# penn-pal-lab/robot_aware_control

Hardware: AMD Instinct MI355X
Metric: SVG train frames/sec + CEM candidate-rollouts/sec, 64x64 (higher is better)
Workload: dtype fp32 (conv operands as two fp16 parts = 22 significant bits, fp32 accumulate; see fp32_exact)

## Files before the change

### include/rac_hip.h

```cpp
#ifndef RAC_HIP_H
#define RAC_HIP_H

#include <stddef.h>
#include <stdint.h>

#ifdef __cplusplus
extern "C" {
#endif

#define RAC_OK 0
#define RAC_EINVAL (-1)
#define RAC_ELAUNCH (-2)

#define RAC_ABI_VERSION 12

int rac_version(void);
const char* rac_device_arch(void);
const char* rac_last_error(void);

enum {
  RAC_CONV_FWD = 0,
  RAC_CONV_DGRAD = 1,
  RAC_CONV_WGRAD = 2
};
// ... 41 lines not shown
typedef struct rac_frag_job {
  const float* w;
  const uint32_t* w_amax;
  uint16_t* parts;
  int64_t part_stride;
  int32_t Cout, Cin, ksize, transposed;
  int64_t block_begin;
} rac_frag_job;
int64_t rac_absmax_blocks(int64_t n);
int64_t rac_weight_frag_blocks(int32_t Cout, int32_t Cin, int32_t ksize);
int rac_absmax_multi(const rac_absmax_job* jobs, int32_t n_jobs, int64_t total_blocks, void* stream);
int rac_weight_frag_split_multi(const rac_frag_job* jobs, int32_t n_jobs, int64_t total_blocks, void* stream);
int rac_conv2d_split_supported(int32_t H, int32_t W, int32_t ksize, int32_t Cin, int32_t Cout, int32_t a_split);
int rac_conv2d_fwd_split(const rac_conv_args* a, const uint32_t* a_amax0, const uint32_t* a_amax1,
                         int64_t w_part_stride, int32_t w_cin, const uint32_t* w_amax, uint32_t* out_amax, void* stream);
int rac_conv2d_fwd_split_pool_ok(const rac_conv_args* a, int32_t w_cin);
int rac_convlstm_cell_fwd_split(const rac_conv_args* a, const uint32_t* a_amax0, const uint32_t* a_amax1,
                                int64_t w_part_stride, int32_t w_cin, const uint32_t* w_amax, const float* c_prev,
                                float* h_out, float* c_out, void* stream);

#define RAC_WGRAD_MAX_STEPS 16
typedef struct rac_wgrad_args {
  int32_t B, H, W;
  int32_t ksize, Cin, Cout, a_split;
  int32_t T;
  int32_t nsplit;
  int32_t accumulate;
  const float* dy[RAC_WGRAD_MAX_STEPS];
  const float* x0[RAC_WGRAD_MAX_STEPS];
  const float* x1[RAC_WGRAD_MAX_STEPS];
// ... 287 lines not shown
```

### robot_aware_control_amd/_lib.py

```python
from __future__ import annotations

import ctypes as C
import os

import torch

_HERE = os.path.dirname(os.path.abspath(__file__))
LIB_PATH = os.environ.get("RAC_HIP_LIB") or os.path.join(_HERE, "librac_hip.so")

i32, i64, f32, vp = C.c_int32, C.c_int64, C.c_float, C.c_void_p


class ConvArgs(C.Structure):
    _fields_ = [
        ("mode", i32), ("B", i32), ("H", i32), ("W", i32), ("ksize", i32), ("Cin", i32), ("Cout", i32),
        ("act", i32), ("split_k", i32), ("accumulate", i32), ("a_split", i32), ("o_split", i32),
        ("slab_stride", i64),
        ("a0", vp), ("a1", vp), ("w", vp), ("out0", vp), ("out1", vp),
        ("bias", vp), ("scale", vp), ("shift", vp), ("stats", vp),
        ("stats_rows", i64), ("a0_up", i32), ("amax_per_image", i32),
    ]


WGRAD_MAX_STEPS = 16
# ... 66 lines not shown
        ("all_ky", i32), ("col_segments", i32),
    ]


_SIGS = {
    "rac_conv2d": [C.POINTER(ConvArgs), vp],
    "rac_absmax": [vp, i64, vp, i64, vp, vp],
    "rac_absmax_rows": [vp, i64, i64, vp, vp],
    "rac_weight_frag_split": [vp, vp, vp, i32, i32, i32, i32, i64, vp],
    "rac_absmax_blocks": [i64],
    "rac_weight_frag_blocks": [i32, i32, i32],
    "rac_absmax_multi": [vp, i32, i64, vp],
    "rac_weight_frag_split_multi": [vp, i32, i64, vp],
    "rac_conv2d_split_supported": [i32, i32, i32, i32, i32, i32],
    "rac_conv2d_fwd_split": [C.POINTER(ConvArgs), vp, vp, i64, i32, vp, vp, vp],
    "rac_conv2d_fwd_split_pool_ok": [C.POINTER(ConvArgs), i32],
    "rac_convlstm_cell_fwd_split": [C.POINTER(ConvArgs), vp, vp, i64, i32, vp, vp, vp, vp, vp],
    "rac_conv2d_wgrad_split": [C.POINTER(WgradArgs), vp],
    "rac_split_steps": [C.POINTER(vp), C.POINTER(vp), i32, i64, C.POINTER(vp), i32, vp],
    "rac_slab_accumulate": [vp, i32, i64, vp, i64, vp],
    "rac_bn_finalize": [vp, i64, vp, vp, vp, vp, f32, f32, i32, vp, vp, vp, vp, i32, i32, vp],
    "rac_affine_act": [vp, vp, vp, i32, vp, i64, i32, i32, vp, vp],
    "rac_bn_apply_act": [vp, i64, vp, vp, vp, vp, f32, f32, i32, vp, i32, vp, vp, vp, vp, vp, i64, i32, i32, vp, vp],
    "rac_bn_bwd_reduce": [vp, vp, vp, vp, vp, vp, vp, i64, i32, i32, vp],
    "rac_bn_bwd_apply": [vp, vp, vp, vp, vp, vp, vp, vp, vp, vp, i64, i32, i32, vp, vp],
    "rac_maxpool2_fwd": [vp, vp, i32, i32, i32, i32, vp],
    "rac_maxpool2_bwd": [vp, vp, vp, i32, i32, i32, i32, vp],
    "rac_upsample2_fwd": [vp, vp, i32, i32, i32, i32, vp],
    "rac_upsample2_bwd": [vp, vp, i32, i32, i32, i32, vp],
    "rac_tilecat_fwd": [vp, i32, vp, i32, vp, i32, vp, i32, vp, i32, i32, vp, i32, i32, vp, i32, vp],
# ... 134 lines not shown
```

### robot_aware_control_amd/csrc/rac_split16.hip

```cpp
#include <math.h>
#include <stdlib.h>

#include <type_traits>

#include "rac_common.h"

namespace rac {

typedef _Float16 f16x8 __attribute__((ext_vector_type(8)));
typedef _Float16 f16x4 __attribute__((ext_vector_type(4)));
typedef unsigned int u32x4 __attribute__((ext_vector_type(4)));
typedef unsigned int u32x2 __attribute__((ext_vector_type(2)));
typedef __amdgpu_buffer_rsrc_t rsrc_t;

constexpr unsigned OOB = 0xFFFFFFF0u;
constexpr int SBN = 128, SBK = 32;

__device__ __forceinline__ const void* uniform_ptr(const void* p) {
  unsigned long long v = reinterpret_cast<unsigned long long>(p);
  unsigned lo = __builtin_amdgcn_readfirstlane((unsigned)v);
  unsigned hi = __builtin_amdgcn_readfirstlane((unsigned)(v >> 32));
  return reinterpret_cast<const void*>(((unsigned long long)hi << 32) | lo);
}
__device__ __forceinline__ rsrc_t make_rsrc(const void* p, unsigned bytes) {
// ... 45 lines not shown
  double* stats;
  long stats_rows;
  int M, N, HW, P, taps, cchunks, nchunks, cps;
  int w_nchunks;
  int xcd_group;
  int tile_m;
  int n_store;
  int a0_up;
  const float* lstm_c_prev;
  float *lstm_h, *lstm_c;
  int lstm_g;
  int per_image;
  int seg_w, seg_h, seg_tx, seg_tpi;
  float* pool_out;
  int pool_bpr;
};

struct SegOrigin {
  int img, y0, x0, m0;
};
__device__ __forceinline__ SegOrigin seg_origin(const Conv16P& p, int bx) {
  SegOrigin o;
  o.img = bx / p.seg_tpi;
  const int r = bx - o.img * p.seg_tpi;
  const int ty = r / p.seg_tx;
  o.y0 = ty * p.seg_h;
  o.x0 = (r - ty * p.seg_tx) * p.seg_w;
  o.m0 = (o.img * p.H + o.y0) * p.W + o.x0;
  return o;
}
// ... 86 lines not shown
        const float sc = pre ? pre[nb][1] : (p.scale ? p.scale[ncol0 + nb * 16 + lr] : 1.f);
        const float sh = pre ? pre[nb][2] : (p.scale ? p.shift[ncol0 + nb * 16 + lr] : 0.f);
#pragma unroll
        for (int r = 0; r < 4; ++r) {
          float v = acc[mb][nb][r] * iav[mb][r] * iw + bias;
          v = v * sc + sh;
          v = v > 0.f ? v : slope * v;
          if (SIG) v = sigmoid_acc(v);
          __builtin_amdgcn_raw_buffer_store_b32(__builtin_bit_cast(unsigned, v), dst, (int)voff[r] + nb * 64, 0, 0);
          mxb[mb] = max(mxb[mb], absbits(v));
        }
      }
    }
    return;
  }
#pragma unroll
  for (int nb = 0; nb < NBLK; ++nb) {
    const int n = ncol0 + nb * 16 + lr;
    const bool nok = n < NS;
    const int nc = nok ? n : 0;
    const float bias = pre ? pre[nb][0] : (p.bias ? p.bias[nc] : 0.f);
    const float sc = pre ? pre[nb][1] : (p.scale ? p.scale[nc] : 1.f);
    const float sh = pre ? pre[nb][2] : (p.scale ? p.shift[nc] : 0.f);
    float s1 = 0.f, s2 = 0.f;
#pragma unroll
    for (int mb = 0; mb < MBLK; ++mb) {
      if (mb0 + mb >= nmb) continue;
#pragma unroll
      for (int r = 0; r < 4; ++r) {
        const int rl = 4 * lq + r;
        const int m = ym_hw ? m0 + (rl >> 3) * ym_hw + (mb0 + mb) * 8 + (rl & 7) : seg_row_pixel(p, m0, (mb0 + mb) * 16) + rl;
        const bool ok = nok & (m < p.M);
        float v = acc[mb][nb][r] * iav[mb][r] * iw + bias;
        const float vs = ok ? v : 0.f;
        s1 += vs;
        s2 += vs * vs;
        v = v * sc + sh;
        v = v > 0.f ? v : slope * v;
        if (SIG) v = sigmoid_acc(v);
        if (ok) {
          p.out0[(long)m * NS + n] = v;
          mxb[mb] = max(mxb[mb], absbits(v));
        }
      }
    }
    if (p.stats) {
      s1 += __shfl_xor(s1, 16);
      s2 += __shfl_xor(s2, 16);
      s1 += __shfl_xor(s1, 32);
      s2 += __shfl_xor(s2, 32);
      if (lq == 0 && nok) {
        double* sg = p.stats + (p.stats_rows ? (long)(m0 / p.stats_rows) * 2 * NS : 0L);
        atomicAdd(sg + n, (double)s1);
        atomicAdd(sg + NS + n, (double)s2);
      }
    }
  }
}

template <int MBLK, int NBLK>
__device__ __forceinline__ void conv16_epilogue(const Conv16P& p, const f32x4 (&acc)[MBLK][NBLK], int m0, int mb0, int nmb,
                                                int ncol0, int bz, float ia, float iw, const float (*pre)[3] = nullptr,
                                                const float* ia_rows = nullptr, unsigned* out_amax = nullptr,
                                                int ym_hw = 0) {
  const int lane = threadIdx.x & 63, lr = lane & 15, lq = lane >> 4;
  const int NS = p.n_store;
  if (p.split_k > 1) {
    float* dst = p.out0 + (long)bz * p.slab_stride;
#pragma unroll
    for (int nb = 0; nb < NBLK; ++nb) {
      const int n = ncol0 + nb * 16 + lr;
#pragma unroll
      for (int mb = 0; mb < MBLK; ++mb) {
        if (mb0 + mb >= nmb) continue;
#pragma unroll
        for (int r = 0; r < 4; ++r) {
          const int rl = 4 * lq + r;
          const int m = ym_hw ? m0 + (rl >> 3) * ym_hw + (mb0 + mb) * 8 + (rl & 7) : seg_row_pixel(p, m0, (mb0 + mb) * 16) + rl;
          if ((n < NS) & (m < p.M)) dst[(long)m * NS + n] = acc[mb][nb][r] * ia * iw;
        }
      }
    }
    return;
  }
  unsigned mxb[MBLK];
  if (p.act == RAC_ACT_SIGMOID)
    conv16_epilogue_body<1>(p, acc, m0, mb0, nmb, ncol0, ia, iw, pre, ia_rows, mxb, ym_hw);
  else
    conv16_epilogue_body<0>(p, acc, m0, mb0, nmb, ncol0, ia, iw, pre, ia_rows, mxb, ym_hw);
  if (!out_amax) return;
  if (ia_rows && ym_hw) {
    unsigned mx = 0;
#pragma unroll
    for (int mb = 0; mb < MBLK; ++mb) mx = max(mx, mxb[mb]);
    const int img0 = m0 / ym_hw;
    amax_commit(lq < 2 ? mx : 0u, out_amax + img0);
    if (m0 + ym_hw < p.M) amax_commit(lq >= 2 ? mx : 0u, out_amax + img0 + 1);
    return;
  }
// ... 1201 lines not shown
          __syncthreads();
          cur ^= 1;
        }
        if (tap < 8 || more) {
#pragma unroll
          for (int t = 0; t < HB; ++t) read_frag(t, (tap + 1) % 9, cur * abuf);
        }
        __builtin_amdgcn_sched_barrier(0);
#pragma unroll
        for (int t = HB; t < MB; ++t)
#pragma unroll
          for (int nb = 0; nb < NB; ++nb) acc[t][nb] = mma3(fa[t], fb[nb], acc[t][nb]);
      }
    }
    const int img = p.per_image ? cur_t.m0 / p.HW : 0;
    conv16_epilogue(p, acc, cur_t.m0, wm * MB, nmb, n0 + wn * NT * 32, 0, pow2f(-cur_t.ka), pow2f(-kw), pre, nullptr,
                    p.out_amax ? p.out_amax + img : nullptr);
    if (!has_next) break;
    cur ^= 1;
    cur_t = nxt_t;
    bx = next_bx;
  }
}

__global__ __launch_bounds__(256) void absmax_kernel(const float4* x0, long n0v, const float4* x1, long n1v,
                                                     unsigned* amax) {
  __shared__ unsigned sh[4];
  unsigned m = 0;
  const long stride = (long)gridDim.x * blockDim.x;
  for (long i = (long)blockIdx.x * blockDim.x + threadIdx.x; i < n0v + n1v; i += stride) {
    const float4 v = i < n0v ? x0[i] : x1[i - n0v];
// ... 882 lines not shown

static int env_int(const char* name, int dflt) {
  const char* e = getenv(name);
  return e ? atoi(e) : dflt;
}

extern "C" int rac_conv2d_split_supported(int32_t H, int32_t W, int32_t ksize, int32_t Cin, int32_t Cout, int32_t a_split) {
  if (H <= 0 || W <= 0 || ksize < 3 || ksize > 5 || !(ksize & 1) || Cin % 32 || Cout % 32) return 0;
  if (a_split > 0 && a_split < Cin && a_split % 32) return 0;
  const int HW = H * W;
  if (HW <= 128) return ((128 / HW) * HW) % 16 == 0;
  if (rows_fit(H, W, ksize)) return 1;
  return ksize == 3 && W >= 64 && W % 16 == 0 && H % 8 == 0;
}

static int conv16_launch(const rac_conv_args* a, const uint32_t* a_amax0, const uint32_t* a_amax1, int64_t w_part_stride,
                         int32_t w_cin, const uint32_t* w_amax, uint32_t* out_amax, const float* lstm_c_prev, float* lstm_h,
                         float* lstm_c, void* stream, bool pool_query = false) {
  RAC_REQUIRE(a && a->mode == RAC_CONV_FWD, "rac_conv2d_fwd_split: forward mode only");
  RAC_REQUIRE(a->B > 0 && a->H > 0 && a->W > 0 && a->Cin > 0 && a->Cout > 0 && a->a0 && a->w && (a->out0 || lstm_h) && a_amax0 &&
                  w_amax,
              "rac_conv2d_fwd_split: bad args");
  const int a_split = (a->a1 && a->a_split > 0 && a->a_split < a->Cin) ? a->a_split : a->Cin;
  const int n_rows = (a->Cout + 31) / 32 * 32;
  RAC_REQUIRE(rac_conv2d_split_supported(a->H, a->W, a->ksize, a->Cin, n_rows, a_split),
              "rac_conv2d_fwd_split: shape not supported (k 3 or 5, channel counts %% 32 == 0, whole images or whole "
              "image rows per 128-pixel tile): use rac_conv2d");
  Conv16P p{};
  p.B = a->B, p.H = a->H, p.W = a->W, p.ks = a->ksize, p.pad = a->ksize / 2;
  p.Cin = a->Cin, p.Cout = a->Cout, p.act = a->act;
  p.split_k = a->split_k > 1 ? a->split_k : 1;
  p.slab_stride = a->slab_stride;
  p.a0 = a->a0, p.a1 = a->a1;
// ... 12 lines not shown
  p.per_image = a->amax_per_image ? 1 : 0;
  RAC_REQUIRE(!p.per_image || (p.split_k == 1 && (p.HW > 128 || p.HW % 16 == 0)),
              "rac_conv2d_fwd_split: amax_per_image needs split_k 1 and H*W a multiple of 16");
  p.lstm_c_prev = lstm_c_prev, p.lstm_h = lstm_h, p.lstm_c = lstm_c, p.lstm_g = a->Cout / 4;
  RAC_REQUIRE(!lstm_h || (lstm_c_prev && lstm_c && a->bias && p.split_k == 1 && p.HW <= 128 && a->Cout % 64 == 0),
              "rac_convlstm_cell_fwd_split: needs c_prev / h / c / bias, split_k 1, a map that fits a tile, 4g % 64 == 0");
  RAC_REQUIRE(!p.a0_up || (p.HW > 128 && a->H % 2 == 0 && a->W % 2 == 0),
              "rac_conv2d_fwd_split: a0_up needs even H, W and a map larger than a 128-pixel tile");
  RAC_REQUIRE(aligned16(a->a0) && aligned16(a->w) && (!a->a1 || aligned16(a->a1)), "rac_conv2d_fwd_split: alignment");
  RAC_REQUIRE((long)p.P * (p.a_split > a->Cin - p.a_split ? p.a_split : a->Cin - p.a_split) * 4 < 0xFFFFFF00L,
              "rac_conv2d_fwd_split: operand larger than 4 GiB");
  if (w_cin <= 0) w_cin = a->Cin;
  RAC_REQUIRE(w_cin >= a->Cin && w_cin % SBK == 0, "rac_conv2d_fwd_split: w_cin must be a multiple of 32, >= Cin");
  RAC_REQUIRE(w_part_stride >= (long)n_rows * p.taps * w_cin && 2 * w_part_stride * 2 < 0xFFFFFF00L,
              "rac_conv2d_fwd_split: weight part stride");
  RAC_REQUIRE(p.split_k == 1 || a->slab_stride >= (long)p.M * p.n_store, "rac_conv2d_fwd_split: slab_stride too small");
  RAC_REQUIRE(p.stats_rows >= 0 && (p.stats_rows == 0 || ((long)a->B * a->H * a->W) % p.stats_rows == 0),
              "rac_conv2d_fwd_split: stats_rows must divide B*H*W");
  p.cchunks = a->Cin / SBK;
  p.nchunks = p.taps * p.cchunks;
  p.w_nchunks = p.taps * (w_cin / SBK);
  p.cps = cdiv(p.nchunks, p.split_k);
  RAC_REQUIRE((long)(n_rows / 32) * p.w_nchunks * 2048L < 0xFFFFFF00L, "rac_conv2d_fwd_split: weight part too large");
  static const bool want_xcd = env_int("RAC_XCD_GROUP", 1);
  if (p.HW > 128) {
    const bool no2d = !env_int("RAC_ROWS_TILE2D", 1);
    const bool fits = rows_fit(a->H, a->W, a->ksize);
    static const int min_w2d = env_int("RAC_ROWS_TILE2D_MINW", 64);
    bool tile2d = a->ksize == 3 && a->W >= min_w2d && a->W % 16 == 0 && a->H % 8 == 0 && !(no2d && fits);
    if (tile2d && p.cps % 9 != 0) {
      if (fits)
        tile2d = false;
// ... 42 lines not shown
    if (fast) {
      fn = fast_fns[width][nv - 2];
      lds_rows = (size_t)2 * 2 * 4 * (((tile2d ? nrows : (nrows / a->W) * (a->W + 2)) + 15) & ~15) * 16;
    }
    {
      const int bpr = (tile2d ? 16 : a->W) / 16, mb_wave = width == 2 ? 2 : 4, bnw = width == 2 ? 32 : (width == 1 ? 64 : 128);
      const bool pool_ok = fast && p.split_k == 1 && !a->stats && !lstm_h && a->H % 2 == 0 && a->W % 16 == 0 &&
                           (bpr == 1 || bpr == 2) && mb_wave % (2 * bpr) == 0 && (p.tile_m / (16 * bpr)) % 2 == 0 &&
                           p.M % p.tile_m == 0 && a->Cout % bnw == 0 && (long)p.M * a->Cout * 4 < (1l << 32);
      if (pool_query) return pool_ok ? 1 : 0;
      if (a->out1) {
        RAC_REQUIRE(pool_ok, "rac_conv2d_fwd_split: this conv cannot pool in its epilogue (rac_conv2d_fwd_split_pool_ok)");
        p.pool_out = a->out1, p.pool_bpr = bpr;
      }
    }
    static bool rows_attr = false;
    if (!rows_attr) {
      for (int i = 0; i < 21; ++i) {
        const rows_fn f = i < 9 ? fns[i / 3][i % 3] : (i < 18 ? fast_fns[(i - 9) / 3][i % 3] : fast5_fns[i - 18]);
        if (f && raise_lds_limit(f, ROWS_LDS_MAX) != RAC_OK) return RAC_ELAUNCH;
      }
      rows_attr = true;
    }
    static const rows_fn persist_fns[2][3] = {
        {conv16_rows_persist_kernel<2, 2, 1>, conv16_rows_persist_kernel<3, 2, 1>, conv16_rows_persist_kernel<4, 2, 1>},
        {conv16_rows_persist_kernel<2, 4, 1>, conv16_rows_persist_kernel<3, 4, 1>, conv16_rows_persist_kernel<4, 4, 1>}};
    static const bool persist = env_int("RAC_ROWS_PERSIST", 1);
    static const int persist_wgs = env_int("RAC_ROWS_PERSIST_WGS", 512);
    if (fast && width >= 1 && p.split_k == 1 && persist &&
        ((int)grid.x >= 32 * persist_wgs || ((int)grid.x >= 4 * persist_wgs && (int)grid.x % persist_wgs == 0))) {
// ... 3 lines not shown
          if (raise_lds_limit(persist_fns[i / 3][i % 3], ROWS_LDS_MAX) != RAC_OK) return RAC_ELAUNCH;
        persist_attr = true;
      }
      static const bool halo = env_int("RAC_PERSIST_HALO_XCD", 1);
      p.xcd_group = (want_xcd && persist_wgs % 8 == 0 && halo) ? 5 : 0;
      hipLaunchKernelGGL(persist_fns[width - 1][nv - 2], dim3(persist_wgs, grid.y, 1), dim3(256), lds_rows,
                         reinterpret_cast<hipStream_t>(stream), p);
      return check_launch("rac_conv2d_fwd_split(image rows, persistent)");
    }
    hipLaunchKernelGGL(fn, grid, dim3(256), lds_rows, reinterpret_cast<hipStream_t>(stream), p);
    return check_launch("rac_conv2d_fwd_split(image rows)");
  }
  if (pool_query) return 0;
  RAC_REQUIRE(!a->out1, "rac_conv2d_fwd_split: maps that fit a tile do not pool in the epilogue");
  p.tile_m = (128 / p.HW) * p.HW;
  RAC_REQUIRE(p.stats_rows % p.tile_m == 0, "rac_conv2d_fwd_split: stats_rows must be a multiple of the tile rows");
  dim3 grid(cdiv(p.M, p.tile_m), cdiv(p.N, SBN), p.split_k);
  p.xcd_group = want_xcd && grid.x > 1 && (grid.y * grid.z) % 8 == 0;
  static const bool pair = env_int("RAC_TILE_PAIR_XCD", 1);
  const bool pair_ok = want_xcd && grid.z == 1 && grid.x >= 64 && pair;
  if (pair_ok && p.xcd_group && grid.y % 8 == 0 && grid.y > 8) p.xcd_group = 3;
  size_t lds_tile = 2 * T16_ABUF;
  static const bool ymajor = env_int("RAC_TILE_YMAJOR", 1);
  const bool ym = a->W == 8 && p.tile_m == 2 * p.HW && ymajor;
  typedef void (*tile_fn)(Conv16P);
  static const bool unroll3 = env_int("RAC_TILE_UNROLL3", 1), unroll5 = env_int("RAC_TILE_UNROLL5", 1);
  const bool u3 = a->ksize == 3 && p.cps % 9 == 0 && unroll3;
  const bool u5 = a->ksize == 5 && p.cps % 25 == 0 && unroll5;
  const tile_fn fn =
      u5 ? (p.tile_m == 128 ? (ym ? (tile_fn)conv16_tile_kernel<2, true, true, 5> : (tile_fn)conv16_tile_kernel<2, true, false, 5>)
                            : (ym ? (tile_fn)conv16_tile_kernel<2, false, true, 5> : (tile_fn)conv16_tile_kernel<2, false, false, 5>)) :
      u3 ? (p.tile_m == 128 ? (ym ? (tile_fn)conv16_tile_kernel<2, true, true, 3> : (tile_fn)conv16_tile_kernel<2, true, false, 3>)
// ... 7 lines not shown
      for (tile_fn f : {(tile_fn)conv16_tile_kernel<2, true, true>, (tile_fn)conv16_tile_kernel<2, false, true>,
                        (tile_fn)conv16_tile_kernel<2, true, true, 3>, (tile_fn)conv16_tile_kernel<2, false, true, 3>,
                        (tile_fn)conv16_tile_kernel<2, true, true, 5>, (tile_fn)conv16_tile_kernel<2, false, true, 5>})
        if (raise_lds_limit(f, 2 * T16Y_ABUF) != RAC_OK) return RAC_ELAUNCH;
      ym_attr = true;
    }
  }
  hipLaunchKernelGGL(fn, grid, dim3(256), lds_tile, reinterpret_cast<hipStream_t>(stream), p);
  return check_launch("rac_conv2d_fwd_split(whole images)");
}

extern "C" int rac_conv2d_fwd_split(const rac_conv_args* a, const uint32_t* a_amax0, const uint32_t* a_amax1,
                                    int64_t w_part_stride, int32_t w_cin, const uint32_t* w_amax, uint32_t* out_amax,
                                    void* stream) {
  return conv16_launch(a, a_amax0, a_amax1, w_part_stride, w_cin, w_amax, out_amax, nullptr, nullptr, nullptr, stream);
}

extern "C" int rac_conv2d_fwd_split_pool_ok(const rac_conv_args* a, int32_t w_cin) {
  static const uint32_t one = 0x3F800000u;
  if (!a || a->mode != RAC_CONV_FWD || !a->a0 || !a->w || !a->out0) return 0;
  const int n_rows = (a->Cout + 31) / 32 * 32;
  const long taps = (long)a->ksize * a->ksize;
  const int r = conv16_launch(a, &one, nullptr, (int64_t)n_rows * taps * (w_cin > 0 ? w_cin : a->Cin), w_cin, &one, nullptr,
                              nullptr, nullptr, nullptr, nullptr, true);
  return r == 1 ? 1 : 0;
}

extern "C" int rac_convlstm_cell_fwd_split(const rac_conv_args* a, const uint32_t* a_amax0, const uint32_t* a_amax1,
                                           int64_t w_part_stride, int32_t w_cin, const uint32_t* w_amax, const float* c_prev,
                                           float* h_out, float* c_out, void* stream) {
// ... 154 lines not shown
```

### robot_aware_control_amd/ops.py

```python
from __future__ import annotations

import contextlib
import ctypes as C
import functools
import os
import weakref
from typing import Optional, Tuple

import torch

from . import _lib
from ._lib import (AbsmaxJob, AdamFragJob, AdamRange, ConvArgs, FragJob, GradSrc, OptimRange, WgradArgs, call, ptr,
                   stream_ptr)

FWD, DGRAD, WGRAD = 0, 1, 2
ACT_NONE, ACT_LEAKY, ACT_SIGMOID = 0, 1, 2
LOSS_KINDS = {"mse": 0, "l1": 1, "dontcare_mse": 2, "dontcare_l1": 3}
BN_EPS, BN_MOMENTUM = 1e-5, 0.1


def _require_cuda(t: torch.Tensor):
    if not t.is_cuda:
        raise _lib.RacError("robot_aware_control_amd ops run on the GPU only (no CPU fallback); got a CPU tensor")

# ... 716 lines not shown
        ent.tag = None
    if ent.tag != _wp_tag(weight):
        gate = PARAM_GATE
        if gate is not None:
            src = getattr(weight, "_rac_pad_source", None)
            base = src[0]() if src is not None else weight
            if base is not None and not gate.ready(base):
                gate.wait_params()
        _wp_refresh(weight.device)
    return ent.parts[transposed], ent.slot


_CONV_ARGS = {}


def _split_launch(x0, x1, a0, a1, pw, wslot, out, *, B, H, W, k, Cin, Cout, C0, act=ACT_NONE, bias=None, scale=None,
                  shift=None, stats=None, split_k=1, slab_stride=0, stats_rows=0, out_amax=None, w_cin=0, a0_up=0,
                  per_image=False, pool=None):
    key = (B, H, W, k, Cin, Cout, act, split_k, C0, slab_stride, stats_rows, a0_up, per_image)
    args = _CONV_ARGS.get(key)
    if args is None:
        args = _CONV_ARGS[key] = ConvArgs(mode=FWD, B=B, H=H, W=W, ksize=k, Cin=Cin, Cout=Cout, act=act, split_k=split_k,
                                          accumulate=0, a_split=C0, o_split=0, slab_stride=slab_stride, stats_rows=stats_rows,
                                          a0_up=a0_up, amax_per_image=1 if per_image else 0)
    args.a0, args.a1, args.w, args.out0 = ptr(x0), ptr(x1), ptr(pw), ptr(out)
    args.out1 = None if isinstance(pool, str) else ptr(pool)
    args.bias, args.scale, args.shift, args.stats = ptr(bias), ptr(scale), ptr(shift), ptr(stats)
    if isinstance(pool, str):
        return bool(_lib.load().rac_conv2d_fwd_split_pool_ok(C.byref(args), w_cin))
    prof = PROFILE
    timed = prof is not None and prof["match"] == (FWD, k, Cin, Cout)
    if timed:
        e0, e1 = torch.cuda.Event(enable_timing=True), torch.cuda.Event(enable_timing=True)
        e0.record()
    if SHAPE_LOG is not None:
        _log_shape("conv16", DGRAD if getattr(pw, "_rac_transposed", False) else FWD, k, B * H * W, Cout, Cin * k * k,
                   2500.0 / 3)
    call("rac_conv2d_fwd_split", C.byref(args), ptr(a0), ptr(a1), pw.shape[1], w_cin, ptr(wslot), ptr(out_amax),
         stream_ptr())
    if timed:
        e1.record()
        prof["events"].append((e0, e1, B * H * W))
        prof["split"] = True


def is_zero(t) -> bool:
    return t is not None and getattr(t, "_rac_zero", False)


def per_image_ok(H: int, W: int) -> bool:
    return H * W > 128 or (H * W) % 16 == 0


SLAB_STATS = os.environ.get("RAC_SLAB_STATS", "1") == "1"
# ... 45 lines not shown
        pooled = torch.empty((B, H // 2, W // 2, Cout), device=x0.device, dtype=torch.float32)
        try:
            _split_launch(x0, x1, a0, a1, pw, wslot, out, act=act, bias=bias, scale=scale, shift=shift, out_amax=slot,
                          pool=pooled if ok else None, **kw)
        except _lib.RacError as e:
            if not ok or "cannot pool" not in str(e):
                raise
            ok = _POOL_OK[key] = False
            _split_launch(x0, x1, a0, a1, pw, wslot, out, act=act, bias=bias, scale=scale, shift=shift, out_amax=slot, **kw)
        if not ok:
            call("rac_maxpool2_fwd", ptr(out), ptr(pooled), B, H, W, Cout, stream_ptr())
        return tag_amax(out, slot), tag_amax(pooled, slot)
    if split == 1:
        _split_launch(x0, x1, a0, a1, pw, wslot, out, act=act, bias=bias, scale=scale, shift=shift, stats=stats,
                      stats_rows=(M // groups if (groups > 1 and stats is not None) else 0), out_amax=slot, **kw)
    else:
        slabs = torch.empty((split, M * Cout), device=x0.device, dtype=torch.float32)
        _split_launch(x0, x1, a0, a1, pw, wslot, slabs, split_k=split, slab_stride=M * Cout, **kw)
        if (SLAB_STATS and stats is not None and bias is None and Cout % 4 == 0 and (Cout // 4) & (Cout // 4 - 1) == 0
                and Cout <= 1024):
            call("rac_slab_reduce_stats", ptr(slabs), split, M * Cout, ptr(out), ptr(stats), M, Cout, groups, ptr(slot),
                 stream_ptr())
            return tag_amax(out, slot)
        call("rac_slab_reduce", ptr(slabs), split, M * Cout, ptr(bias), ptr(out), M * Cout, Cout, ptr(slot),
             stream_ptr())
        if stats is not None:
            call("rac_col_stats", ptr(out), ptr(stats), M, Cout, groups, stream_ptr())
    return tag_amax(out, slot)


# ... 34 lines not shown
    timed = prof is not None and prof["match"] == (FWD, k, Cin, 4 * g)
    if timed:
        e0, e1 = torch.cuda.Event(enable_timing=True), torch.cuda.Event(enable_timing=True)
        e0.record()
    if SHAPE_LOG is not None:
        _log_shape("conv16", FWD, k, B * H * W, 4 * g, Cin * k * k, 2500.0 / 3)
    call("rac_convlstm_cell_fwd_split", C.byref(args), ptr(a0), ptr(a1), pw.shape[1], w_cin, ptr(wslot), ptr(c_prev),
         ptr(h), ptr(c), stream_ptr())
    if timed:
        e1.record()
        prof["events"].append((e0, e1, B * H * W))
        prof["split"] = True
    return h, c


def conv_dgrad_split(dy, weight, C0: int, C1: int = 0, need1: bool = True):
    B, H, W, Cout = dy.shape
    Co, Cin, k, _ = weight.shape
    assert Co == Cout and Cin == C0 + C1
    if C1 and not need1 and C0 % 32 == 0:
        Cin, C1 = C0, 0
    M = B * H * W
    dy = dy if dy.is_contiguous() else dy.contiguous()
    pw, wslot = weight_parts(weight, transposed=True)
    split = plan_split_k(M, Cin, k * k * _cdiv(Cout, 32), tile128_only=True)
    dx0 = torch.empty((B, H, W, C0), device=dy.device, dtype=torch.float32)
    s0 = amax_slot(dy.device)
    if split == 1 and not C1:
        _split_launch(dy, None, amax_for(dy), None, pw, wslot, dx0, B=B, H=H, W=W, k=k, Cin=Cout, Cout=Cin, C0=Cout,
                      out_amax=s0)
        return tag_amax(dx0, s0), None
    slabs = torch.empty((split, M * Cin), device=dy.device, dtype=torch.float32)
    _split_launch(dy, None, amax_for(dy), None, pw, wslot, slabs, B=B, H=H, W=W, k=k, Cin=Cout, Cout=Cin, C0=Cout,
                  split_k=split, slab_stride=M * Cin)
    if C1:
        dx1 = torch.empty((B, H, W, C1), device=dy.device, dtype=torch.float32)
        s1 = amax_slot(dy.device)
        call("rac_slab_reduce2", ptr(slabs), split, M * Cin, None, ptr(dx0), ptr(dx1), M, Cin, C0, ptr(s0), ptr(s1),
             stream_ptr())
        return tag_amax(dx0, s0), tag_amax(dx1, s1)
    call("rac_slab_reduce", ptr(slabs), split, M * Cin, None, ptr(dx0), M * Cin, Cin, ptr(s0), stream_ptr())
    return tag_amax(dx0, s0), None


DEFER_WGRAD = os.environ.get("RAC_DEFER_WGRAD", "1") == "1"
# ... 534 lines not shown
        draw = torch.empty_like(raw)
        want_affine = gamma.requires_grad
        sums = zeros64((G, 2, Cout), dy.device)
        call("rac_bn_bwd_reduce", ptr(dy), ptr(raw), ptr(aff[0]), ptr(aff[1]), ptr(aff[2]), ptr(aff[3]), ptr(sums), M,
             Cout, G, stream_ptr())
        call("rac_bn_bwd_apply", ptr(dy), ptr(raw), ptr(aff[0]), ptr(aff[1]), ptr(aff[2]), ptr(aff[3]), ptr(sums),
             ptr(draw), ptr(grad_buffer(gamma)) if want_affine else None,
             ptr(grad_buffer(beta)) if want_affine else None, M, Cout, G,
             ptr(tag_amax(draw, amax_slot(dy.device))._rac_amax), stream_ptr())
        C0 = x0.shape[3]
        C1 = x1.shape[3] if x1 is not None else 0
        dx0 = dx1 = None
        if ctx.needs_input_grad[0] or (x1 is not None and ctx.needs_input_grad[1]):
            wuse = padded_weight(weight, C0) if ctx.padded else weight
            if ctx.split:
                dx0, dx1 = conv_dgrad_split(draw, wuse, C0, C1)
            else:
                dx0, dx1 = conv_dgrad(draw, wuse, C0, C1)
        if weight.requires_grad:
            Bq, Hq, Wq, _ = draw.shape
            split, padded = ctx.split, ctx.padded

            def wgrad():
                if (padded and x1 is None and weight.shape[1] <= 8 and Cout == 64 and weight.shape[2] == 3
                        and Hq % 16 == 0 and Wq % 16 == 0):
                    thin_wgrad_acc(draw, x0, weight.shape[1], weight)
                elif split:
                    conv_wgrad_split_acc(draw, x0, x1, weight)
                elif padded:
                    wgrad_padded_acc(draw, x0, weight)
                else:
# ... 1501 lines not shown
```

Measured before the change: 4089.

## Reduce split-K partials in-kernel with last-arriving workgroup finishing the epilogue

```diff
diff --git a/include/rac_hip.h b/include/rac_hip.h
--- a/include/rac_hip.h
+++ b/include/rac_hip.h
@@ -79,6 +79,14 @@
 int rac_conv2d_split_supported(int32_t H, int32_t W, int32_t ksize, int32_t Cin, int32_t Cout, int32_t a_split);
 int rac_conv2d_fwd_split(const rac_conv_args* a, const uint32_t* a_amax0, const uint32_t* a_amax1,
                          int64_t w_part_stride, int32_t w_cin, const uint32_t* w_amax, uint32_t* out_amax, void* stream);
+int rac_conv2d_fwd_split_finish(const rac_conv_args* a, const uint32_t* a_amax0, const uint32_t* a_amax1,
+                                int64_t w_part_stride, int32_t w_cin, const uint32_t* w_amax, uint32_t* out_amax,
+                                uint32_t* tile_counters, int64_t n_counters, float* scratch, int64_t scratch_floats,
+                                void* stream);
+int rac_conv2d_dgrad_split_finish(const rac_conv_args* a, const uint32_t* dy_amax, int64_t w_part_stride, int32_t w_cin,
+                                  const uint32_t* w_amax, uint32_t* dx_amax, uint32_t* tile_counters, int64_t n_counters,
+                                  float* scratch, int64_t scratch_floats, void* stream);
+int rac_conv2d_split_finish_size(const rac_conv_args* a, int32_t w_cin, int64_t* n_counters, int64_t* scratch_floats);
 int rac_conv2d_fwd_split_pool_ok(const rac_conv_args* a, int32_t w_cin);
 int rac_convlstm_cell_fwd_split(const rac_conv_args* a, const uint32_t* a_amax0, const uint32_t* a_amax1,
                                 int64_t w_part_stride, int32_t w_cin, const uint32_t* w_amax, const float* c_prev,
diff --git a/robot_aware_control_amd/_lib.py b/robot_aware_control_amd/_lib.py
--- a/robot_aware_control_amd/_lib.py
+++ b/robot_aware_control_amd/_lib.py
@@ -104,6 +104,9 @@
     "rac_weight_frag_split_multi": [vp, i32, i64, vp],
     "rac_conv2d_split_supported": [i32, i32, i32, i32, i32, i32],
     "rac_conv2d_fwd_split": [C.POINTER(ConvArgs), vp, vp, i64, i32, vp, vp, vp],
+    "rac_conv2d_fwd_split_finish": [C.POINTER(ConvArgs), vp, vp, i64, i32, vp, vp, vp, i64, vp, i64, vp],
+    "rac_conv2d_dgrad_split_finish": [C.POINTER(ConvArgs), vp, i64, i32, vp, vp, vp, i64, vp, i64, vp],
+    "rac_conv2d_split_finish_size": [C.POINTER(ConvArgs), i32, vp, vp],
     "rac_conv2d_fwd_split_pool_ok": [C.POINTER(ConvArgs), i32],
     "rac_convlstm_cell_fwd_split": [C.POINTER(ConvArgs), vp, vp, i64, i32, vp, vp, vp, vp, vp],
     "rac_conv2d_wgrad_split": [C.POINTER(WgradArgs), vp],
diff --git a/robot_aware_control_amd/csrc/rac_split16.hip b/robot_aware_control_amd/csrc/rac_split16.hip
--- a/robot_aware_control_amd/csrc/rac_split16.hip
+++ b/robot_aware_control_amd/csrc/rac_split16.hip
@@ -83,6 +83,8 @@
   int seg_w, seg_h, seg_tx, seg_tpi;
   float* pool_out;
   int pool_bpr;
+  unsigned* fin_counters;
+  float* fin_scratch;
 };
 
 struct SegOrigin {
@@ -199,6 +201,7 @@
     }
     return;
   }
+  const bool fine = p.stats && p.stats_rows > 0 && p.stats_rows < p.tile_m;
 #pragma unroll
   for (int nb = 0; nb < NBLK; ++nb) {
     const int n = ncol0 + nb * 16 + lr;
@@ -207,7 +210,7 @@
     const float bias = pre ? pre[nb][0] : (p.bias ? p.bias[nc] : 0.f);
     const float sc = pre ? pre[nb][1] : (p.scale ? p.scale[nc] : 1.f);
     const float sh = pre ? pre[nb][2] : (p.scale ? p.shift[nc] : 0.f);
-    float s1 = 0.f, s2 = 0.f;
+    double s1 = 0., s2 = 0.;
 #pragma unroll
     for (int mb = 0; mb < MBLK; ++mb) {
       if (mb0 + mb >= nmb) continue;
@@ -218,8 +221,8 @@
         const bool ok = nok & (m < p.M);
         float v = acc[mb][nb][r] * iav[mb][r] * iw + bias;
         const float vs = ok ? v : 0.f;
-        s1 += vs;
-        s2 += vs * vs;
+        s1 += (double)vs;
+        s2 += (double)vs * (double)vs;
         v = v * sc + sh;
         v = v > 0.f ? v : slope * v;
         if (SIG) v = sigmoid_acc(v);
@@ -228,28 +231,110 @@
           mxb[mb] = max(mxb[mb], absbits(v));
         }
       }
-    }
-    if (p.stats) {
+      if (fine) {
+        s1 += __shfl_xor(s1, 16);
+        s2 += __shfl_xor(s2, 16);
+        if (!ym_hw) {
+          s1 += __shfl_xor(s1, 32);
+          s2 += __shfl_xor(s2, 32);
+        }
+        const int mrow = ym_hw ? m0 + (lq >> 1) * ym_hw + (mb0 + mb) * 8 : m0 + (mb0 + mb) * 16;
+        if ((ym_hw ? (lq & 1) == 0 : lq == 0) && nok && mrow < p.M) {
+          double* sg = p.stats + (long)(mrow / p.stats_rows) * 2 * NS;
+          atomicAdd(sg + n, s1);
+          atomicAdd(sg + NS + n, s2);
+        }
+        s1 = s2 = 0.;
+      }
+    }
+    if (p.stats && !fine) {
       s1 += __shfl_xor(s1, 16);
       s2 += __shfl_xor(s2, 16);
       s1 += __shfl_xor(s1, 32);
       s2 += __shfl_xor(s2, 32);
       if (lq == 0 && nok) {
         double* sg = p.stats + (p.stats_rows ? (long)(m0 / p.stats_rows) * 2 * NS : 0L);
-        atomicAdd(sg + n, (double)s1);
-        atomicAdd(sg + NS + n, (double)s2);
+        atomicAdd(sg + n, s1);
+        atomicAdd(sg + NS + n, s2);
       }
     }
   }
 }
 
 template <int MBLK, int NBLK>
+__device__ __forceinline__ void conv16_epilogue_fused(const Conv16P& p, const f32x4 (&acc)[MBLK][NBLK], int m0, int mb0,
+                                                      int nmb, int ncol0, float ia, float iw, const float (*pre)[3],
+                                                      const float* ia_rows, unsigned* out_amax, int ym_hw);
+
+template <int MBLK, int NBLK>
+__device__ __forceinline__ bool conv16_finish_gather(const Conv16P& p, const f32x4 (&acc)[MBLK][NBLK],
+                                                     f32x4 (&sum)[MBLK][NBLK], int mb0, int nmb, int bz, float ia, float iw) {
+  __shared__ unsigned fin_ticket;
+  int fin_tile = blockIdx.x + gridDim.x * blockIdx.y;
+  if (p.xcd_group) {
+    const int mt = gridDim.x, nt = gridDim.y;
+    const int lin = blockIdx.x + mt * (blockIdx.y + nt * blockIdx.z);
+    const int xcd = lin & 7, s = lin >> 3;
+    const int grp = (s / mt) * 8 + xcd;
+    fin_tile = s % mt + mt * (grp % nt);
+  }
+  constexpr int WAVE4 = 64 * MBLK * NBLK;
+  constexpr long WG4 = 4L * WAVE4;
+  const f32x4* tile = reinterpret_cast<const f32x4*>(p.fin_scratch) + (long)fin_tile * p.split_k * WG4 +
+                      (threadIdx.x >> 6) * WAVE4 + (threadIdx.x & 63);
+  f32x4* mine = const_cast<f32x4*>(tile) + bz * WG4;
+#pragma unroll
+  for (int mb = 0; mb < MBLK; ++mb) {
+    if (mb0 + mb >= nmb) continue;
+#pragma unroll
+    for (int nb = 0; nb < NBLK; ++nb) mine[(mb * NBLK + nb) * 64] = acc[mb][nb] * ia * iw;
+  }
+  __threadfence();
+  __syncthreads();
+  if (threadIdx.x == 0)
+    fin_ticket = __hip_atomic_fetch_add(p.fin_counters + fin_tile, 1u, __ATOMIC_ACQ_REL, __HIP_MEMORY_SCOPE_AGENT);
+  __syncthreads();
+  if (fin_ticket != (unsigned)(p.split_k - 1)) return false;
+  __threadfence();
+  if (threadIdx.x == 0) __hip_atomic_store(p.fin_counters + fin_tile, 0u, __ATOMIC_RELAXED, __HIP_MEMORY_SCOPE_AGENT);
+#pragma unroll
+  for (int mb = 0; mb < MBLK; ++mb) {
+    const bool live = mb0 + mb < nmb;
+#pragma unroll
+    for (int nb = 0; nb < NBLK; ++nb) sum[mb][nb] = live ? tile[(mb * NBLK + nb) * 64] : f32x4{0.f, 0.f, 0.f, 0.f};
+  }
+  for (int s = 1; s < p.split_k; ++s) {
+    tile += WG4;
+    f32x4 part[MBLK][NBLK];
+#pragma unroll
+    for (int mb = 0; mb < MBLK; ++mb) {
+      const bool live = mb0 + mb < nmb;
+#pragma unroll
+      for (int nb = 0; nb < NBLK; ++nb) part[mb][nb] = live ? tile[(mb * NBLK + nb) * 64] : f32x4{0.f, 0.f, 0.f, 0.f};
+    }
+#pragma unroll
+    for (int mb = 0; mb < MBLK; ++mb)
+#pragma unroll
+      for (int nb = 0; nb < NBLK; ++nb) sum[mb][nb] += part[mb][nb];
+  }
+  return true;
+}
+
+template <bool FIN = true, int MBLK, int NBLK>
 __device__ __forceinline__ void conv16_epilogue(const Conv16P& p, const f32x4 (&acc)[MBLK][NBLK], int m0, int mb0, int nmb,
                                                 int ncol0, int bz, float ia, float iw, const float (*pre)[3] = nullptr,
                                                 const float* ia_rows = nullptr, unsigned* out_amax = nullptr,
                                                 int ym_hw = 0) {
   const int lane = threadIdx.x & 63, lr = lane & 15, lq = lane >> 4;
   const int NS = p.n_store;
+  if constexpr (FIN) {
+    if (p.split_k > 1 && p.fin_counters) {
+      f32x4 sum[MBLK][NBLK];
+      if (!conv16_finish_gather(p, acc, sum, mb0, nmb, bz, ia, iw)) return;
+      conv16_epilogue_fused(p, sum, m0, mb0, nmb, ncol0, 1.f, 1.f, pre, ia_rows, out_amax, ym_hw);
+      return;
+    }
+  }
   if (p.split_k > 1) {
     float* dst = p.out0 + (long)bz * p.slab_stride;
 #pragma unroll
@@ -268,6 +353,14 @@
     }
     return;
   }
+  conv16_epilogue_fused(p, acc, m0, mb0, nmb, ncol0, ia, iw, pre, ia_rows, out_amax, ym_hw);
+}
+
+template <int MBLK, int NBLK>
+__device__ __forceinline__ void conv16_epilogue_fused(const Conv16P& p, const f32x4 (&acc)[MBLK][NBLK], int m0, int mb0,
+                                                      int nmb, int ncol0, float ia, float iw, const float (*pre)[3],
+                                                      const float* ia_rows, unsigned* out_amax, int ym_hw) {
+  const int lane = threadIdx.x & 63, lq = lane >> 4;
   unsigned mxb[MBLK];
   if (p.act == RAC_ACT_SIGMOID)
     conv16_epilogue_body<1>(p, acc, m0, mb0, nmb, ncol0, ia, iw, pre, ia_rows, mxb, ym_hw);
@@ -1499,7 +1592,7 @@
       }
     }
     const int img = p.per_image ? cur_t.m0 / p.HW : 0;
-    conv16_epilogue(p, acc, cur_t.m0, wm * MB, nmb, n0 + wn * NT * 32, 0, pow2f(-cur_t.ka), pow2f(-kw), pre, nullptr,
+    conv16_epilogue<false>(p, acc, cur_t.m0, wm * MB, nmb, n0 + wn * NT * 32, 0, pow2f(-cur_t.ka), pow2f(-kw), pre, nullptr,
                     p.out_amax ? p.out_amax + img : nullptr);
     if (!has_next) break;
     cur ^= 1;
@@ -2412,9 +2505,31 @@
   return ksize == 3 && W >= 64 && W % 16 == 0 && H % 8 == 0;
 }
 
+struct Conv16Finish {
+  uint32_t* counters;
+  int64_t n_counters;
+  float* scratch;
+  int64_t scratch_floats;
+  int64_t* need;
+};
+
+static int conv16_finish_setup(Conv16P& p, const Conv16Finish* fin, dim3 grid, int acc_blocks) {
+  const int64_t tiles = (int64_t)grid.x * grid.y;
+  const int64_t floats = tiles * p.split_k * 256 * acc_blocks * 4;
+  if (fin->need) {
+    fin->need[0] = tiles, fin->need[1] = floats;
+    return RAC_OK;
+  }
+  RAC_REQUIRE(fin->counters && fin->scratch && aligned16(fin->scratch), "rac_conv2d_split_finish: null or unaligned arena");
+  RAC_REQUIRE(tiles <= fin->n_counters && floats <= fin->scratch_floats,
+              "rac_conv2d_split_finish: arena too small (rac_conv2d_split_finish_size)");
+  p.fin_counters = fin->counters, p.fin_scratch = fin->scratch;
+  return RAC_OK;
+}
+
 static int conv16_launch(const rac_conv_args* a, const uint32_t* a_amax0, const uint32_t* a_amax1, int64_t w_part_stride,
                          int32_t w_cin, const uint32_t* w_amax, uint32_t* out_amax, const float* lstm_c_prev, float* lstm_h,
-                         float* lstm_c, void* stream, bool pool_query = false) {
+                         float* lstm_c, void* stream, bool pool_query = false, const Conv16Finish* fin = nullptr) {
   RAC_REQUIRE(a && a->mode == RAC_CONV_FWD, "rac_conv2d_fwd_split: forward mode only");
   RAC_REQUIRE(a->B > 0 && a->H > 0 && a->W > 0 && a->Cin > 0 && a->Cout > 0 && a->a0 && a->w && (a->out0 || lstm_h) && a_amax0 &&
                   w_amax,
@@ -2457,8 +2572,9 @@
   RAC_REQUIRE(w_cin >= a->Cin && w_cin % SBK == 0, "rac_conv2d_fwd_split: w_cin must be a multiple of 32, >= Cin");
   RAC_REQUIRE(w_part_stride >= (long)n_rows * p.taps * w_cin && 2 * w_part_stride * 2 < 0xFFFFFF00L,
               "rac_conv2d_fwd_split: weight part stride");
-  RAC_REQUIRE(p.split_k == 1 || a->slab_stride >= (long)p.M * p.n_store, "rac_conv2d_fwd_split: slab_stride too small");
-  RAC_REQUIRE(p.stats_rows >= 0 && (p.stats_rows == 0 || ((long)a->B * a->H * a->W) % p.stats_rows == 0),
+  RAC_REQUIRE(p.split_k == 1 || fin || a->slab_stride >= (long)p.M * p.n_store, "rac_conv2d_fwd_split: slab_stride too small");
+  RAC_REQUIRE(!fin || (p.split_k > 1 && a->out0 && !a->out1 && !lstm_h && !p.per_image),
+              "rac_conv2d_split_finish: needs split_k > 1 and out0; no pooled output, cell epilogue or per-image scales");  RAC_REQUIRE(p.stats_rows >= 0 && (p.stats_rows == 0 || ((long)a->B * a->H * a->W) % p.stats_rows == 0),
               "rac_conv2d_fwd_split: stats_rows must divide B*H*W");
   p.cchunks = a->Cin / SBK;
   p.nchunks = p.taps * p.cchunks;
@@ -2531,6 +2647,10 @@
         p.pool_out = a->out1, p.pool_bpr = bpr;
       }
     }
+    if (fin) {
+      const int r = conv16_finish_setup(p, fin, grid, width == 0 ? 16 : (width == 1 ? 8 : 4));
+      if (r != RAC_OK || fin->need) return r;
+    }
     static bool rows_attr = false;
     if (!rows_attr) {
       for (int i = 0; i < 21; ++i) {
@@ -2564,8 +2684,13 @@
   if (pool_query) return 0;
   RAC_REQUIRE(!a->out1, "rac_conv2d_fwd_split: maps that fit a tile do not pool in the epilogue");
   p.tile_m = (128 / p.HW) * p.HW;
-  RAC_REQUIRE(p.stats_rows % p.tile_m == 0, "rac_conv2d_fwd_split: stats_rows must be a multiple of the tile rows");
+  RAC_REQUIRE(p.stats_rows % p.tile_m == 0 || (p.stats_rows % p.HW == 0 && p.tile_m % p.stats_rows == 0 && p.HW % 16 == 0),
+              "rac_conv2d_fwd_split: stats_rows must be a multiple of the tile rows, or whole images that divide a tile");
   dim3 grid(cdiv(p.M, p.tile_m), cdiv(p.N, SBN), p.split_k);
+  if (fin) {
+    const int r = conv16_finish_setup(p, fin, grid, 16);
+    if (r != RAC_OK || fin->need) return r;
+  }
   p.xcd_group = want_xcd && grid.x > 1 && (grid.y * grid.z) % 8 == 0;
   static const bool pair = env_int("RAC_TILE_PAIR_XCD", 1);
   const bool pair_ok = want_xcd && grid.z == 1 && grid.x >= 64 && pair;
@@ -2603,6 +2728,40 @@
                                     int64_t w_part_stride, int32_t w_cin, const uint32_t* w_amax, uint32_t* out_amax,
                                     void* stream) {
   return conv16_launch(a, a_amax0, a_amax1, w_part_stride, w_cin, w_amax, out_amax, nullptr, nullptr, nullptr, stream);
+}
+
+extern "C" int rac_conv2d_fwd_split_finish(const rac_conv_args* a, const uint32_t* a_amax0, const uint32_t* a_amax1,
+                                           int64_t w_part_stride, int32_t w_cin, const uint32_t* w_amax, uint32_t* out_amax,
+                                           uint32_t* tile_counters, int64_t n_counters, float* scratch,
+                                           int64_t scratch_floats, void* stream) {
+  const Conv16Finish fin{tile_counters, n_counters, scratch, scratch_floats, nullptr};
+  return conv16_launch(a, a_amax0, a_amax1, w_part_stride, w_cin, w_amax, out_amax, nullptr, nullptr, nullptr, stream, false,
+                       &fin);
+}
+
+extern "C" int rac_conv2d_dgrad_split_finish(const rac_conv_args* a, const uint32_t* dy_amax, int64_t w_part_stride,
+                                             int32_t w_cin, const uint32_t* w_amax, uint32_t* dx_amax,
+                                             uint32_t* tile_counters, int64_t n_counters, float* scratch,
+                                             int64_t scratch_floats, void* stream) {
+  RAC_REQUIRE(a && !a->a1 && !a->bias && !a->scale && !a->stats && a->act == RAC_ACT_NONE,
+              "rac_conv2d_dgrad_split_finish: one source (dy), no bias / scale / activation / statistics");
+  const Conv16Finish fin{tile_counters, n_counters, scratch, scratch_floats, nullptr};
+  return conv16_launch(a, dy_amax, nullptr, w_part_stride, w_cin, w_amax, dx_amax, nullptr, nullptr, nullptr, stream, false,
+                       &fin);
+}
+
+extern "C" int rac_conv2d_split_finish_size(const rac_conv_args* a, int32_t w_cin, int64_t* n_counters,
+                                            int64_t* scratch_floats) {
+  static const uint32_t one = 0x3F800000u;
+  RAC_REQUIRE(a && n_counters && scratch_floats, "rac_conv2d_split_finish_size: null argument");
+  const int n_rows = (a->Cout + 31) / 32 * 32;
+  const long taps = (long)a->ksize * a->ksize;
+  int64_t need[2] = {0, 0};
+  const Conv16Finish fin{nullptr, 0, nullptr, 0, need};
+  const int r = conv16_launch(a, &one, nullptr, (int64_t)n_rows * taps * (w_cin > 0 ? w_cin : a->Cin), w_cin, &one, nullptr,
+                              nullptr, nullptr, nullptr, nullptr, false, &fin);
+  *n_counters = need[0], *scratch_floats = need[1];
+  return r;
 }
 
 extern "C" int rac_conv2d_fwd_split_pool_ok(const rac_conv_args* a, int32_t w_cin) {
diff --git a/robot_aware_control_amd/ops.py b/robot_aware_control_amd/ops.py
--- a/robot_aware_control_amd/ops.py
+++ b/robot_aware_control_amd/ops.py
@@ -754,9 +754,39 @@
 _CONV_ARGS = {}
 
 
+FINISH_MIN_COUNTERS = 4096
+_FINISH_ARENA = {}
+_FINISH_NEED = {}
+
+
+def finish_in_launch(M: int, N: int, nchunks: int, split: int) -> bool:
+    return _finish_rule(M, N, nchunks, split, os.environ.get("RAC_SPLIT_FINISH", "auto"))
+
+
+@functools.lru_cache(maxsize=None)
+def _finish_rule(M, N, nchunks, split, mode):
+    if split <= 1 or mode == "0":
+        return False
+    if mode == "1":
+        return True
+    return True
+
+
+def finish_arena(device, n_counters: int, scratch_floats: int):
+    key = (device.index, stream_ptr())
+    arena = _FINISH_ARENA.get(key)
+    if arena is None:
+        arena = _FINISH_ARENA[key] = [None, None]
+    if arena[0] is None or arena[0].numel() < n_counters:
+        arena[0] = torch.zeros(max(FINISH_MIN_COUNTERS, n_counters), device=device, dtype=torch.int32)
+    if arena[1] is None or arena[1].numel() < scratch_floats:
+        arena[1] = torch.empty(scratch_floats, device=device, dtype=torch.float32)
+    return arena
+
+
 def _split_launch(x0, x1, a0, a1, pw, wslot, out, *, B, H, W, k, Cin, Cout, C0, act=ACT_NONE, bias=None, scale=None,
                   shift=None, stats=None, split_k=1, slab_stride=0, stats_rows=0, out_amax=None, w_cin=0, a0_up=0,
-                  per_image=False, pool=None):
+                  per_image=False, pool=None, finish=None):
     key = (B, H, W, k, Cin, Cout, act, split_k, C0, slab_stride, stats_rows, a0_up, per_image)
     args = _CONV_ARGS.get(key)
     if args is None:
@@ -776,8 +806,22 @@
     if SHAPE_LOG is not None:
         _log_shape("conv16", DGRAD if getattr(pw, "_rac_transposed", False) else FWD, k, B * H * W, Cout, Cin * k * k,
                    2500.0 / 3)
-    call("rac_conv2d_fwd_split", C.byref(args), ptr(a0), ptr(a1), pw.shape[1], w_cin, ptr(wslot), ptr(out_amax),
-         stream_ptr())
+    if finish:
+        need = _FINISH_NEED.get(key)
+        if need is None:
+            buf = (C.c_int64 * 2)()
+            call("rac_conv2d_split_finish_size", C.byref(args), w_cin, C.addressof(buf), C.addressof(buf) + 8)
+            need = _FINISH_NEED[key] = (int(buf[0]), int(buf[1]))
+        counters, scratch = finish_arena(x0.device, *need)
+        if finish == "dgrad":
+            call("rac_conv2d_dgrad_split_finish", C.byref(args), ptr(a0), pw.shape[1], w_cin, ptr(wslot), ptr(out_amax),
+                 ptr(counters), counters.numel(), ptr(scratch), scratch.numel(), stream_ptr())
+        else:
+            call("rac_conv2d_fwd_split_finish", C.byref(args), ptr(a0), ptr(a1), pw.shape[1], w_cin, ptr(wslot),
+                 ptr(out_amax), ptr(counters), counters.numel(), ptr(scratch), scratch.numel(), stream_ptr())
+    else:
+        call("rac_conv2d_fwd_split", C.byref(args), ptr(a0), ptr(a1), pw.shape[1], w_cin, ptr(wslot), ptr(out_amax),
+             stream_ptr())
     if timed:
         e1.record()
         prof["events"].append((e0, e1, B * H * W))
@@ -853,6 +897,9 @@
     if split == 1:
         _split_launch(x0, x1, a0, a1, pw, wslot, out, act=act, bias=bias, scale=scale, shift=shift, stats=stats,
                       stats_rows=(M // groups if (groups > 1 and stats is not None) else 0), out_amax=slot, **kw)
+    elif stats is not None and bias is None and finish_in_launch(M, Cout, k * k * _cdiv(Cin, 32), split):
+        _split_launch(x0, x1, a0, a1, pw, wslot, out, split_k=split, stats=stats,
+                      stats_rows=(M // groups if groups > 1 else 0), out_amax=slot, finish="fwd", **kw)
     else:
         slabs = torch.empty((split, M * Cout), device=x0.device, dtype=torch.float32)
         _split_launch(x0, x1, a0, a1, pw, wslot, slabs, split_k=split, slab_stride=M * Cout, **kw)
@@ -917,7 +964,7 @@
     return h, c
 
 
-def conv_dgrad_split(dy, weight, C0: int, C1: int = 0, need1: bool = True):
+def conv_dgrad_split(dy, weight, C0: int, C1: int = 0, need1: bool = True, vgg: bool = False):
     B, H, W, Cout = dy.shape
     Co, Cin, k, _ = weight.shape
     assert Co == Cout and Cin == C0 + C1
@@ -932,6 +979,10 @@
     if split == 1 and not C1:
         _split_launch(dy, None, amax_for(dy), None, pw, wslot, dx0, B=B, H=H, W=W, k=k, Cin=Cout, Cout=Cin, C0=Cout,
                       out_amax=s0)
+        return tag_amax(dx0, s0), None
+    if vgg and not C1 and finish_in_launch(M, Cin, k * k * _cdiv(Cout, 32), split):
+        _split_launch(dy, None, amax_for(dy), None, pw, wslot, dx0, B=B, H=H, W=W, k=k, Cin=Cout, Cout=Cin, C0=Cout,
+                      split_k=split, out_amax=s0, finish="dgrad")
         return tag_amax(dx0, s0), None
     slabs = torch.empty((split, M * Cin), device=dy.device, dtype=torch.float32)
     _split_launch(dy, None, amax_for(dy), None, pw, wslot, slabs, B=B, H=H, W=W, k=k, Cin=Cout, Cout=Cin, C0=Cout,
@@ -1496,7 +1547,7 @@
         if ctx.needs_input_grad[0] or (x1 is not None and ctx.needs_input_grad[1]):
             wuse = padded_weight(weight, C0) if ctx.padded else weight
             if ctx.split:
-                dx0, dx1 = conv_dgrad_split(draw, wuse, C0, C1)
+                dx0, dx1 = conv_dgrad_split(draw, wuse, C0, C1, vgg=True)
             else:
                 dx0, dx1 = conv_dgrad(draw, wuse, C0, C1)
         if weight.requires_grad:
```

Result: slower. 3539 (-13.4%).
